# nico-bohlinger/RL-X

Measured on AMD Instinct MI355X. Metric: env-steps/sec (whole node) PPO 4096 envs at 1/2/4/8 MI355X, higher is better.
Workload: dtype f32

## Files before the change

### rl-x_amd/csrc/common.h

```cpp
#pragma once
#include <hip/hip_runtime.h>
#include <hip/hip_ext.h>
#include <stdint.h>
#include <cstring>
#include <cmath>
#include <string>
#include <vector>
#include <functional>
#include "../../include/rlx_hip.h"

namespace rlx {

void set_error(const std::string& msg);

#define RLX_HIP_TRY(expr)                                                                      \
  do {                                                                                         \
    hipError_t e_ = (expr);                                                                    \
    if (e_ != hipSuccess) {                                                                    \
      ::rlx::set_error(std::string(#expr) + " failed: " + hipGetErrorString(e_) + " (" __FILE__ \
                       ":" + std::to_string(__LINE__) + ")");                                  \
      return RLX_EHIP;                                                                         \
    }                                                                                          \
  } while (0)

// ... 37 lines not shown
  hipEvent_t e0, e1;
};
struct ProfRow {
  int kid, engine;
  int64_t M;
  int N, K;
  int64_t launches, timed;
  double ms, flops, bytes;
};
struct Twin { const void* p[4] = {nullptr, nullptr, nullptr, nullptr}; };

}

struct AttrOnce {
  uint64_t mask = 0;
  static int dev() { int d = 0; (void)hipGetDevice(&d); return d & 63; }
  bool done() const { return (mask >> dev()) & 1; }
  void mark() { mask |= 1ull << dev(); }
};

struct rlx_ctx {
  int device = 0;
  rlx::Scratch slots[3][rlx::SL_COUNT];
  int bank = 0;
  int opt_flip = 0;
  hipStream_t side = nullptr;
  hipEvent_t ev_fork = nullptr, ev_join = nullptr;
  hipEvent_t ev_rows[2] = {nullptr, nullptr};
  hipEvent_t ev_cdone[2] = {nullptr, nullptr};
  const float* dbg_sac_eps[2] = {nullptr, nullptr};
  bool l1fwd_mfma = true;
  bool pipeline_updates = true;
  bool pf_valid = false;
  uint32_t pf_key_in[2] = {0, 0}, pf_key_out[2] = {0, 0};
  int pf_E = 0, pf_scheme = 0;
  int64_t pf_B = 0;
  hipEvent_t pf_done = nullptr;
  hipEvent_t ev_perm_free = nullptr;
  bool perm_free_recorded = false;
  bool two_streams = true;
  const uint32_t* l1_xmax = nullptr;
  const uint32_t* xmax_slot[2] = {nullptr, nullptr};
  int lf_idle_cus = 0;
  bool dw_recompute = false;
  float* l12_stats = nullptr;
  bool l12_ran = false;
  bool dw_merge = true;
  void* dbg_stamps = nullptr;
  bool fwd2h = true;
  int gather_group_rows = 524288;
  bool gather_records = true;
  bool l12_fused = true;
  int ppo_tail = -1;
  int ppo_twin = -1;
  bool fused_recurrent_act = true;
  int num_cus = 256;
  void* defer = nullptr;
  bool prof_on = false;
  int prof_sample = 1;
  hipEvent_t prof_ref = nullptr;
  double prof_union_ms = 0.0;
  std::vector<rlx::ProfRec> prof_recs;
  std::vector<rlx::ProfRow> prof_rows;
  std::vector<hipEvent_t> prof_pool;
  bool gemm_bx = true;
  float bx_gscale = 1.f;
  bool adam_emit = true;
  bool bx_keep[3] = {false, false, false};
  struct RoImages { bool valid = false; const float* params[2] = {nullptr, nullptr}; const void* img[2][3] = {}; int nt[2][3] = {}; } ro_img;
  int bx_force_mi = 0;
  int bx_debug = 0;
  struct BxImage { const float* W; int trans, K, N; const void* img; };
  BxImage bx_img[3][32];
  int bx_n[3] = {0, 0, 0};
  bool disable_l1fused = false;
  std::vector<char> ro_nets_shadow;
  int rank = 0, world = 1;
  void* comm = nullptr;
  hipStream_t comm_stream = nullptr;
  hipEvent_t comm_ev[32] = {};
  int comm_ev_pos = 0;
  rlx_allreduce_fn ar_hook = nullptr;
  void* ar_hook_user = nullptr;
  int ro_exit = 0;
  int64_t bx_window_fallbacks = 0;
  int64_t ar_calls = 0;
  hipStream_t sac_st[2] = {nullptr, nullptr};
  hipEvent_t sac_ev[6] = {nullptr, nullptr, nullptr, nullptr, nullptr, nullptr};
  struct SacImages {
    bool valid = false; const float *pp = nullptr, *qp = nullptr, *qt = nullptr; rlx_mlp_desc pd{}, qd{}; int64_t np = 0, nq2 = 0;
    void written(const float* p, int64_t n) {
      if (!valid) return;
      auto hit = [&](const float* b, int64_t m) { return b && p < b + m && b < p + n; };
      if (hit(pp, np) || hit(qp, nq2) || hit(qt, nq2)) valid = false;
    }
  } sac_img;
  const void* sac_img_arena = nullptr;
  int sac_twin = 1;
  float* sched_host[4] = {nullptr, nullptr, nullptr, nullptr};
  hipEvent_t sched_ev[4] = {nullptr, nullptr, nullptr, nullptr};
  size_t sched_cap = 0;
  int sched_pos = 0;
  int espo_chunk = 2;
  int32_t* espo_host = nullptr;
  hipEvent_t espo_ev[3] = {nullptr, nullptr, nullptr};
  bool pf_dist = false;
// ... 329 lines not shown
```

### rl-x_amd/csrc/core.hip

```cpp
#include "common.h"
#include <algorithm>
#include <cstdio>
#include <cstdlib>
#include <utility>

namespace rlx {

static thread_local std::string g_last_error;

void set_error(const std::string& msg) { g_last_error = msg; }

void* scratch(rlx_ctx* ctx, ScratchSlot s, size_t bytes) {
  Scratch& sl = ctx->slots[ctx->bank][s];
  if (sl.bytes >= bytes && sl.ptr) return sl.ptr;
  if (sl.ptr) {
    if (hipDeviceSynchronize() != hipSuccess) { set_error("hipDeviceSynchronize failed in scratch()"); return nullptr; }
    (void)hipFree(sl.ptr);
    sl.ptr = nullptr;
    sl.bytes = 0;
  }
  size_t want = ((bytes > (size_t(1) << 20) ? bytes + bytes / 8 : bytes) + 255) & ~size_t(255);
  void* p = nullptr;
  hipError_t e = hipMalloc(&p, want);
  if (e != hipSuccess) {
// ... 153 lines not shown
      if (q.engine != rlx::PROF_ENGINE_HBM && ctx->prof_ref && hipEventElapsedTime(&t0, ctx->prof_ref, r.e0) == hipSuccess)
        iv.emplace_back(t0, t0 + ms);
    }
    ctx->prof_pool.push_back(r.e0);
    ctx->prof_pool.push_back(r.e1);
  }
  ctx->prof_recs.clear();
  std::sort(iv.begin(), iv.end());
  double uni = 0.0;
  float cs = 0.f, ce = -1.f;
  for (auto& p : iv) {
    if (ce < 0.f || p.first > ce) { if (ce >= 0.f) uni += ce - cs; cs = p.first; ce = p.second; }
    else if (p.second > ce) ce = p.second;
  }
  if (ce >= 0.f) uni += ce - cs;
  ctx->prof_union_ms = uni;
  return RLX_OK;
}

int rlx_prof_rows(rlx_ctx* ctx, rlx_prof_row* rows, int capacity, int* n_out) {
  RLX_REQUIRE(ctx && n_out && (rows || capacity == 0), RLX_EINVAL, "rlx_prof_rows: NULL pointer");
  const int n = (int)ctx->prof_rows.size();
  *n_out = n;
  for (int i = 0; i < n && i < capacity; ++i) {
    const rlx::ProfRow& q = ctx->prof_rows[i];
    rows[i] = rlx_prof_row{q.kid, q.engine, q.N, q.K, q.M, q.launches, q.timed, q.ms, q.flops, q.bytes};
  }
  return RLX_OK;
}

int rlx_prof_union_ms(rlx_ctx* ctx, double* out) {
  RLX_REQUIRE(ctx && out, RLX_EINVAL, "rlx_prof_union_ms: NULL pointer");
  *out = ctx->prof_union_ms;
  return RLX_OK;
}

int rlx_dbg_set_option(rlx_ctx* ctx, const char* name, int value) {
  RLX_REQUIRE(ctx && name, RLX_EINVAL, "rlx_dbg_set_option: NULL");
  if (std::string(name) == "sac_twin") { ctx->sac_twin = value; return RLX_OK; }
  if (std::string(name) == "disable_l1fused") { ctx->disable_l1fused = value != 0; return RLX_OK; }
  if (std::string(name) == "l1fwd_mfma") { ctx->l1fwd_mfma = value != 0; return RLX_OK; }
  if (std::string(name) == "pipeline_updates") { ctx->pipeline_updates = value != 0; return RLX_OK; }
  if (std::string(name) == "two_streams") { ctx->two_streams = value != 0; return RLX_OK; }
  if (std::string(name) == "ppo_twin") { ctx->ppo_twin = value; return RLX_OK; }
  if (std::string(name) == "ro_exit") { ctx->ro_exit = value; return RLX_OK; }
  if (std::string(name) == "lf_idle_cus") { ctx->lf_idle_cus = value < 0 ? 0 : value; return RLX_OK; }
  if (std::string(name) == "dw_recompute") { ctx->dw_recompute = value != 0; return RLX_OK; }
  if (std::string(name) == "dw_merge") { ctx->dw_merge = value != 0; return RLX_OK; }
  if (std::string(name) == "fwd2h") { ctx->fwd2h = value != 0; return RLX_OK; }
  if (std::string(name) == "l12_fused") { ctx->l12_fused = value != 0; return RLX_OK; }
  if (std::string(name) == "gather_group_rows") { ctx->gather_group_rows = value; return RLX_OK; }
  if (std::string(name) == "gather_records") { ctx->gather_records = value != 0; return RLX_OK; }
  if (std::string(name) == "ppo_tail") { ctx->ppo_tail = value < 0 ? -1 : (value > 2 ? 2 : value); return RLX_OK; }
  if (std::string(name) == "bx_force_mi") { ctx->bx_force_mi = value; return RLX_OK; }
  if (std::string(name) == "adam_emit") { ctx->adam_emit = value != 0; return RLX_OK; }
  if (std::string(name) == "bx_debug") { ctx->bx_debug = value; return RLX_OK; }
  if (std::string(name) == "bx_gscale_log2") { ctx->bx_gscale = ldexpf(1.f, value < 0 ? 0 : (value > 40 ? 40 : value)); return RLX_OK; }
  if (std::string(name) == "gemm_bx") { ctx->gemm_bx = value != 0; return RLX_OK; }
  if (std::string(name) == "prof_sample") { ctx->prof_sample = value < 1 ? 1 : value; return RLX_OK; }
  if (std::string(name) == "espo_chunk") { ctx->espo_chunk = value < 1 ? 1 : value; return RLX_OK; }
  if (std::string(name) == "fused_recurrent_act") { ctx->fused_recurrent_act = value != 0; return RLX_OK; }
  RLX_REQUIRE(false, RLX_EINVAL, "rlx_dbg_set_option: unknown option");
}

int rlx_dbg_get_counter(rlx_ctx* ctx, const char* name, int64_t* out) {
  RLX_REQUIRE(ctx && name && out, RLX_EINVAL, "rlx_dbg_get_counter: NULL");
  int bank = 0, slot = 0;
  if (sscanf(name, "scratch_ptr:%d:%d", &bank, &slot) == 2 && bank >= 0 && bank < 3 && slot >= 0 && slot < rlx::SL_COUNT) {
    *out = (int64_t)reinterpret_cast<uintptr_t>(ctx->slots[bank][slot].ptr);
    return RLX_OK;
  }
  if (sscanf(name, "scratch_bytes:%d:%d", &bank, &slot) == 2 && bank >= 0 && bank < 3 && slot >= 0 && slot < rlx::SL_COUNT) {
    *out = (int64_t)ctx->slots[bank][slot].bytes;
    return RLX_OK;
  }
  if (std::string(name) == "allreduce_calls") { *out = ctx->ar_calls; return RLX_OK; }
  if (std::string(name) == "bx_window_fallbacks") { *out = ctx->bx_window_fallbacks; return RLX_OK; }
  if (std::string(name) == "gemm_bx") { *out = ctx->gemm_bx ? 1 : 0; return RLX_OK; }
  RLX_REQUIRE(false, RLX_EINVAL, "rlx_dbg_get_counter: unknown counter");
}

int rlx_version(void) { return 200; }

const char* rlx_last_error(void) { return rlx::g_last_error.c_str(); }

int rlx_ctx_create(int device, rlx_ctx** out) {
  RLX_REQUIRE(out != nullptr, RLX_EINVAL, "rlx_ctx_create: out is NULL");
  int count = 0;
  RLX_HIP_TRY(hipGetDeviceCount(&count));
  RLX_REQUIRE(device >= 0 && device < count, RLX_EINVAL, "rlx_ctx_create: no such HIP device");
  RLX_HIP_TRY(hipSetDevice(device));
  hipDeviceProp_t prop;
  RLX_HIP_TRY(hipGetDeviceProperties(&prop, device));
  rlx_ctx* c = new rlx_ctx();
  c->device = device;
  c->num_cus = prop.multiProcessorCount;
  if (const char* e = getenv("RLX_GEMM_BX")) c->gemm_bx = atoi(e) != 0;
  if (const char* e = getenv("RLX_BX_DEBUG")) c->bx_debug = atoi(e);
  *out = c;
  return RLX_OK;
}

int rlx_dist_release(rlx_ctx* ctx);

int rlx_ctx_destroy(rlx_ctx* ctx) {
  if (!ctx) return RLX_OK;
// ... 40 lines not shown
```

### rl-x_amd/csrc/ppo.hip

```cpp
#include "ppo_internal.h"
#include "gemm_bx.h"
#include "dist.h"

namespace rlx {

constexpr float LOG_2PI = 1.8378770664093453f;
constexpr float HALF_LOG_2PIE = 1.4189385332046727f;
constexpr int HEAD_ROWS = 64;

__global__ __launch_bounds__(256) void k_gather(const float* __restrict__ states, const float* __restrict__ actions,
                                                const float* __restrict__ logp, const float* __restrict__ returns,
                                                const float* __restrict__ adv, const int32_t* __restrict__ idx,
                                                float* __restrict__ mb_x, float* __restrict__ mb_a,
                                                float* __restrict__ aux, const int32_t* __restrict__ valid_rows,
                                                int64_t mb, int O, int A, const float* __restrict__ cstates,
                                                float* __restrict__ mb_xc, int Oc) {
  const int64_t nv = valid_rows ? (int64_t)*valid_rows : mb;
  const int64_t nx = mb * O, na = mb * A, nxc = cstates ? mb * Oc : 0;
  const int64_t total = nx + na + mb + nxc;
  for (int64_t e = (int64_t)blockIdx.x * 256 + threadIdx.x; e < total; e += (int64_t)gridDim.x * 256) {
    if (e >= nx + na + mb) {
      const int64_t f = e - nx - na - mb;
      const int64_t r = f / Oc;
      const int d = (int)(f - r * Oc);
// ... 837 lines not shown
    }
  }
  __syncthreads();
  {
    constexpr int nk3 = K / X_BK;
    auto loadT = [&](int kt, float4 (&rr)[2]) {
      const int kk = (kt < nk3 ? kt : nk3 - 1) * X_BK;
#pragma unroll
      for (int p = 0; p < 2; ++p) rr[p] = *reinterpret_cast<const float4*>(T + (a_r + 32 * p) * TL_TS + kk + a_c);
    };
    const float so2 = X_WINV / gs;
    const int ntc = N2 / G_BN;
    for (int nt = 0; nt < ntc; ++nt) {
      f32x16 acc[1][2];
#pragma unroll
      for (int j = 0; j < 2; ++j)
#pragma unroll
        for (int rr = 0; rr < 16; ++rr) acc[0][j][rr] = 0.f;
      bx_kloop<1>(planes, n.W3t, nk3, ntc * 4, nt * 4 + wn * 2, wm, lane, a_r, a_c, loadT, acc, gs);
      const int64_t off = (m0 + wm * 32 + 4 * (lane >> 5)) * N2 + nt * G_BN + wn * 64 + (lane & 31);
      const float* hsb = n.H2 + off;
      float* cb = n.dZ2 + off;
      float hh[2][16];
#pragma unroll
      for (int j = 0; j < 2; ++j)
#pragma unroll
        for (int rr = 0; rr < 16; ++rr) hh[j][rr] = hsb[(int64_t)((rr & 3) + 8 * (rr >> 2)) * N2 + j * 32];
#pragma unroll
      for (int j = 0; j < 2; ++j)
#pragma unroll
        for (int rr = 0; rr < 16; ++rr)
          cb[(int64_t)((rr & 3) + 8 * (rr >> 2)) * N2 + j * 32] = acc[0][j][rr] * so2 * act_grad_t<ACT>(hh[j][rr]);
    }
  }
}

template <int ACT>
__global__ __launch_bounds__(256, 2) void k_tail_bx(TailNet p, TailNet c, const float* __restrict__ mb_a,
                                                    const float* __restrict__ aux, const double* __restrict__ stats,
                                                    float* __restrict__ metrics, int64_t M, int N2, float inv_mb, float clip,
                                                    float ent_coef, float critic_coef, const int32_t* __restrict__ valid_rows,
                                                    float gs, int both, int which) {
  extern __shared__ __attribute__((aligned(16))) char tl_smem[];
  const bool critic = both ? blockIdx.y != 0 : which != 0;
  if (!critic)
    tail_body<true, ACT>(p, tl_smem, mb_a, aux, stats, metrics, M, N2, inv_mb, clip, ent_coef, critic_coef, valid_rows, gs);
  else
    tail_body<false, ACT>(c, tl_smem, mb_a, aux, stats, metrics, M, N2, inv_mb, clip, ent_coef, critic_coef, valid_rows, gs);
}

#ifndef RLX_T32_PFC
#define RLX_T32_PFC 2
#endif
constexpr int T32_ROWS = 32;
template <bool POLICY, int ACT, int N2>
__device__ __forceinline__ void tail32_body(const TailNet& n, char* __restrict__ smem, const float* __restrict__ mb_a,
                                            const float* __restrict__ aux, const double* __restrict__ stats,
                                            float* __restrict__ metrics, int64_t M, float inv_mb, float clip, float ent_coef,
                                            float critic_coef, const int32_t* __restrict__ valid_rows, float gs) {
  constexpr int K = TL_K3, AP = 8, NP = 2, RP = T32_ROWS / NP, KQ = K / 8;
  constexpr int HROW = 2 * N2 + 16, HPL = T32_ROWS * HROW;
  constexpr int DROW = 2 * K + 16, DPL = T32_ROWS * DROW;
  constexpr int TREG = (T32_ROWS * TL_TS * 4 > 2 * DPL) ? T32_ROWS * TL_TS * 4 : 2 * DPL;
  char* H2P = smem;
  float* T = reinterpret_cast<float*>(smem + 2 * HPL);
  char* D3P = smem + 2 * HPL;
  float* Ws = reinterpret_cast<float*>(smem + 2 * HPL + TREG);
  float* Ds = Ws + K * AP;
  float* DLs = Ds + T32_ROWS * AP;
  float* red = DLs + T32_ROWS * AP;
  const int t = threadIdx.x, lane = t & 63, w = t >> 6, li = lane & 31, lh = lane >> 5;
  const int64_t m0 = (int64_t)blockIdx.x * T32_ROWS;
  const int A = n.A, PS = n.PS;
  {
    constexpr int NV = T32_ROWS * N2 / 4 / 256;
    float4 hv[NV];
    const int sr = t >> 3, sc = (t & 7) * 4;
    const float* hp = n.H2 + (m0 + sr) * N2 + sc;
#pragma unroll
    for (int i = 0; i < NV; ++i) hv[i] = *reinterpret_cast<const float4*>(hp + 32 * i);
    for (int i = t; i < K * AP; i += 256) {
      const int k = i >> 3, a = i & 7;
      Ws[i] = a < A ? n.Wh[k * A + a] : 0.f;
    }
    char* d0 = H2P + sr * HROW + sc * 2;
#pragma unroll
    for (int i = 0; i < NV; ++i) {
      uint32_t a0, a1, b0, b1;
      bx_split2(hv[i].x * X_ASCALE, hv[i].y * X_ASCALE, a0, a1);
      bx_split2(hv[i].z * X_ASCALE, hv[i].w * X_ASCALE, b0, b1);
      *reinterpret_cast<u32x2*>(d0 + 64 * i) = u32x2{a0, b0};
      *reinterpret_cast<u32x2*>(d0 + 64 * i + HPL) = u32x2{a1, b1};
    }
  }
  __syncthreads();
  {
    f32x16 acc;
#pragma unroll
    for (int r = 0; r < 16; ++r) acc[r] = 0.f;
    constexpr int NB = N2 / 16, PF = 4;
    const char* ard = H2P + li * HROW + lh * 16;
    const u32x4* wf = n.W3f + (int64_t)w * X_NP * 64 + lane;
    constexpr int wstep = 4 * X_NP * 64;
    u32x4 bq[PF][X_NP];
#pragma unroll
    for (int u = 0; u < PF; ++u)
#pragma unroll
      for (int p = 0; p < X_NP; ++p) bq[u][p] = wf[(int64_t)u * wstep + p * 64];
#define T32_BLOCK(QU, REFILL)                                                                                         \
  {                                                                                                                   \
    u32x4 av[X_NP];                                                                                                   \
    _Pragma("unroll") for (int p = 0; p < X_NP; ++p) av[p] = *reinterpret_cast<const u32x4*>(ard + (QU) * 32 + p * HPL); \
    acc = __builtin_amdgcn_mfma_f32_32x32x16_f16(__builtin_bit_cast(f16x8, av[0]), __builtin_bit_cast(f16x8, bq[u][1]), acc, 0, 0, 0); \
    acc = __builtin_amdgcn_mfma_f32_32x32x16_f16(__builtin_bit_cast(f16x8, av[1]), __builtin_bit_cast(f16x8, bq[u][0]), acc, 0, 0, 0); \
    acc = __builtin_amdgcn_mfma_f32_32x32x16_f16(__builtin_bit_cast(f16x8, av[0]), __builtin_bit_cast(f16x8, bq[u][0]), acc, 0, 0, 0); \
    if (REFILL) {                                                                                                     \
      _Pragma("unroll") for (int p = 0; p < X_NP; ++p) bq[u][p] = wf[(int64_t)((QU) + PF) * wstep + p * 64];           \
    }                                                                                                                 \
    __builtin_amdgcn_sched_barrier(0);                                                                                \
  }
#pragma unroll 1
    for (int q = 0; q < NB - PF; q += PF) {
#pragma unroll
      for (int u = 0; u < PF; ++u) T32_BLOCK(q + u, true)
    }
#pragma unroll
    for (int u = 0; u < PF; ++u) T32_BLOCK(NB - PF + u, false)
#undef T32_BLOCK
    const float so = X_AINV * X_WINV, bv = n.b3[w * 32 + li];
    float* tb = T + (4 * lh) * TL_TS + w * 32 + li;
#pragma unroll
    for (int r = 0; r < 16; ++r) tb[((r & 3) + 8 * (r >> 2)) * TL_TS] = act_fwd_t<ACT>(fmaf(acc[r], so, bv));
  }
  __syncthreads();
  const int r = t >> 3, q8 = t & 7;
  const int64_t row = m0 + r;
  const bool valid = row < (valid_rows ? (int64_t)*valid_rows : M);
  float bias[AP], ls[AP];
#pragma unroll
  for (int a = 0; a < AP; ++a) {
    bias[a] = a < A ? n.bh[a] : 0.f;
    ls[a] = (POLICY && a < A) ? n.logstd[a] : 0.f;
  }
  hl_f4 h[KQ / 4];
  {
    const hl_f4* hp = reinterpret_cast<const hl_f4*>(T + r * TL_TS + q8 * KQ);
#pragma unroll
    for (int j = 0; j < KQ / 4; ++j) h[j] = hp[j];
  }
  float out[AP];
#pragma unroll
  for (int a = 0; a < AP; ++a) out[a] = 0.f;
#pragma unroll
  for (int j = 0; j < KQ / 4; ++j)
#pragma unroll
    for (int e = 0; e < 4; ++e) {
      const float* wr = Ws + (q8 * KQ + 4 * j + e) * AP;
      const hl_f4 w0 = *reinterpret_cast<const hl_f4*>(wr), w1 = *reinterpret_cast<const hl_f4*>(wr + 4);
      const float hv = h[j][e];
#pragma unroll
      for (int a = 0; a < 4; ++a) { out[a] = fmaf(hv, w0[a], out[a]); out[4 + a] = fmaf(hv, w1[a], out[4 + a]); }
    }
#pragma unroll
  for (int a = 0; a < AP; ++a) {
    out[a] += dpp_f(out[a], 0);
    out[a] += dpp_f(out[a], 1);
    out[a] += dpp_f(out[a], 2);
    out[a] += bias[a];
  }
  float d[AP], m0s = 0.f, m1s = 0.f, m2s = 0.f;
#pragma unroll
  for (int a = 0; a < AP; ++a) d[a] = 0.f;
  if (POLICY) {
    float nlp = 0.f, zs[AP], isd[AP];
#pragma unroll
    for (int a = 0; a < AP; ++a) {
      isd[a] = 1.0f / expf(ls[a]);
      const float act_a = (valid && a < A) ? mb_a[row * A + a] : out[a];
      zs[a] = (act_a - out[a]) * isd[a];
      if (a < A) nlp += -0.5f * zs[a] * zs[a] - 0.5f * LOG_2PI - ls[a];
    }
    float amean, ainv, astd;
    adv_norm_from_stats(stats, amean, ainv, astd);
    const float logp_old = valid ? aux[row * 3 + 0] : 0.f;
    const float advn = valid ? (aux[row * 3 + 2] - amean) * ainv : 0.f;
    const float logratio = valid ? nlp - logp_old : 0.f;
    const float ratio = expf(logratio);
    const float pg1 = -advn * ratio;
    const float rc = fminf(fmaxf(ratio, 1.f - clip), 1.f + clip);
    const float pg2 = -advn * rc;
    const bool inside = (ratio >= 1.f - clip) && (ratio <= 1.f + clip);
    const float d_ratio = (inside || pg1 > pg2) ? -advn : 0.f;
    const float d_logp = valid ? d_ratio * ratio * inv_mb : 0.f;
#pragma unroll
    for (int a = 0; a < AP; ++a) {
      d[a] = a < A ? d_logp * zs[a] * isd[a] : 0.f;
      if (q8 == 0) DLs[r * AP + a] = a < A ? d_logp * (zs[a] * zs[a] - 1.f) - (valid ? ent_coef * inv_mb : 0.f) : 0.f;
    }
    if (valid && q8 == 0) {
      m0s = fmaxf(pg1, pg2);
      m1s = (ratio - 1.f) - logratio;
      m2s = fabsf(ratio - 1.f) > clip ? 1.f : 0.f;
    }
    if (blockIdx.x == 0 && t == 0) {
      float ent = 0.f, sstd = 0.f;
      for (int a = 0; a < A; ++a) { ent += ls[a] + HALF_LOG_2PIE; sstd += expf(ls[a]); }
      metrics[2] = ent;
      metrics[5] = amean;
      metrics[6] = astd;
      metrics[7] = sstd / (float)A;
    }
  } else {
    if (valid) {
      const float diff = out[0] - aux[row * 3 + 1];
      if (q8 == 0) m0s = 0.5f * diff * diff;
      d[0] = critic_coef * inv_mb * diff;
    }
  }
  if (q8 == 0) {
#pragma unroll
    for (int a = 0; a < AP; ++a) Ds[r * AP + a] = d[a];
  }
  m0s = wave_sum(m0s);
  m1s = wave_sum(m1s);
  m2s = wave_sum(m2s);
  if ((t & 63) == 0) { red[(t >> 6) * 4 + 0] = m0s; red[(t >> 6) * 4 + 1] = m1s; red[(t >> 6) * 4 + 2] = m2s; }
  __syncthreads();
  float* pw = n.partials + (int64_t)blockIdx.x * PS;
  if (t == 0) {
    float* pm = pw + K * A + 2 * A;
    pm[0] = (red[0] + red[4]) + (red[8] + red[12]);
    pm[1] = (red[1] + red[5]) + (red[9] + red[13]);
    pm[2] = (red[2] + red[6]) + (red[10] + red[14]);
  }
  __syncthreads();
  {
    const int k = t % K, part = t / K;
    float dw[AP];
#pragma unroll
    for (int a = 0; a < AP; ++a) dw[a] = 0.f;
    for (int rr = part * RP; rr < (part + 1) * RP; ++rr) {
      const float hv = T[rr * TL_TS + k];
      const hl_f4 d0 = *reinterpret_cast<const hl_f4*>(Ds + rr * AP), d1 = *reinterpret_cast<const hl_f4*>(Ds + rr * AP + 4);
#pragma unroll
      for (int a = 0; a < 4; ++a) { dw[a] = fmaf(hv, d0[a], dw[a]); dw[4 + a] = fmaf(hv, d1[a], dw[4 + a]); }
    }
#pragma unroll
    for (int a = 0; a < AP; ++a) red[(part * K + k) * AP + a] = dw[a];
    __syncthreads();
    if (part == 0) {
#pragma unroll
      for (int a = 0; a < AP; ++a) dw[a] += red[(K + k) * AP + a];
      for (int a = 0; a < A; ++a) pw[k * A + a] = dw[a];
    }
  }
  if (t < A) {
    float sb = 0.f, sl = 0.f;
    for (int rr = 0; rr < T32_ROWS; ++rr) {
      sb += Ds[rr * AP + t];
      if (POLICY) sl += DLs[rr * AP + t];
    }
    pw[K * A + t] = sb;
    pw[K * A + A + t] = sl;
  }
  __syncthreads();
  {
    hl_f4* gp = reinterpret_cast<hl_f4*>(n.dZ3 + row * K + q8 * KQ);
    char* dp = D3P + r * DROW + q8 * KQ * 2;
#pragma unroll
    for (int j = 0; j < KQ / 4; ++j) {
      hl_f4 o;
#pragma unroll
      for (int e = 0; e < 4; ++e) {
        const float* wr = Ws + (q8 * KQ + 4 * j + e) * AP;
        const hl_f4 w0 = *reinterpret_cast<const hl_f4*>(wr), w1 = *reinterpret_cast<const hl_f4*>(wr + 4);
        float sacc = 0.f;
#pragma unroll
        for (int a = 0; a < 4; ++a) { sacc = fmaf(d[a], w0[a], sacc); sacc = fmaf(d[4 + a], w1[a], sacc); }
        o[e] = sacc * act_grad_t<ACT>(h[j][e]);
      }
      gp[j] = o;
      uint32_t a0, a1, b0, b1;
      bx_split2(o[0] * gs, o[1] * gs, a0, a1);
      bx_split2(o[2] * gs, o[3] * gs, b0, b1);
      *reinterpret_cast<u32x2*>(dp + 8 * j) = u32x2{a0, b0};
      *reinterpret_cast<u32x2*>(dp + 8 * j + DPL) = u32x2{a1, b1};
    }
  }
  __syncthreads();
  {
    constexpr int NTC = N2 / 32, JW = NTC / 4;
    f32x16 acc[JW];
#pragma unroll
    for (int j = 0; j < JW; ++j)
#pragma unroll
      for (int rr = 0; rr < 16; ++rr) acc[j][rr] = 0.f;
    const char* ard = D3P + li * DROW + lh * 16;
    const u32x4* wt = n.W3t + (int64_t)(w * JW) * X_NP * 64 + lane;
    constexpr int wstep = NTC * X_NP * 64;
    constexpr int PFC = RLX_T32_PFC, NBC = K / 16;
    u32x4 bc[PFC][JW][X_NP];
#pragma unroll
    for (int u = 0; u < PFC; ++u)
#pragma unroll
      for (int j = 0; j < JW; ++j)
#pragma unroll
        for (int p = 0; p < X_NP; ++p) bc[u][j][p] = wt[(int64_t)u * wstep + (j * X_NP + p) * 64];
#define T32C_BLOCK(QU, REFILL)                                                                                        \
  {                                                                                                                   \
    u32x4 av[X_NP];                                                                                                   \
    _Pragma("unroll") for (int p = 0; p < X_NP; ++p) av[p] = *reinterpret_cast<const u32x4*>(ard + (QU) * 32 + p * DPL); \
    _Pragma("unroll") for (int j = 0; j < JW; ++j) {                                                                  \
      acc[j] = __builtin_amdgcn_mfma_f32_32x32x16_f16(__builtin_bit_cast(f16x8, av[0]), __builtin_bit_cast(f16x8, bc[u][j][1]), acc[j], 0, 0, 0); \
      acc[j] = __builtin_amdgcn_mfma_f32_32x32x16_f16(__builtin_bit_cast(f16x8, av[1]), __builtin_bit_cast(f16x8, bc[u][j][0]), acc[j], 0, 0, 0); \
      acc[j] = __builtin_amdgcn_mfma_f32_32x32x16_f16(__builtin_bit_cast(f16x8, av[0]), __builtin_bit_cast(f16x8, bc[u][j][0]), acc[j], 0, 0, 0); \
    }                                                                                                                 \
    if (REFILL) {                                                                                                     \
      _Pragma("unroll") for (int j = 0; j < JW; ++j) _Pragma("unroll") for (int p = 0; p < X_NP; ++p)                  \
          bc[u][j][p] = wt[(int64_t)((QU) + PFC) * wstep + (j * X_NP + p) * 64];                                       \
    }                                                                                                                 \
    __builtin_amdgcn_sched_barrier(0);                                                                                \
  }
    static_assert(NBC % PFC == 0 && NBC >= PFC, "phase C: whole groups of PFC blocks");
#pragma unroll 1
    for (int q = 0; q < NBC - PFC; q += PFC) {
#pragma unroll
      for (int u = 0; u < PFC; ++u) T32C_BLOCK(q + u, true)
    }
#pragma unroll
    for (int u = 0; u < PFC; ++u) T32C_BLOCK(NBC - PFC + u, false)
#undef T32C_BLOCK
    const float so2 = X_WINV / gs;
#pragma unroll
    for (int j = 0; j < JW; ++j) {
      const int col = (w * JW + j) * 32 + li;
      float* cb = n.dZ2 + (m0 + 4 * lh) * N2 + col;
      const char* hb = H2P + (4 * lh) * HROW + col * 2;
#pragma unroll
      for (int rr = 0; rr < 16; ++rr) {
        const int rho = (rr & 3) + 8 * (rr >> 2);
        const _Float16 hi = *reinterpret_cast<const _Float16*>(hb + rho * HROW);
        const _Float16 lo = *reinterpret_cast<const _Float16*>(hb + rho * HROW + HPL);
        const float h2 = ((float)hi + (float)lo) * X_AINV;
        cb[(int64_t)rho * N2] = acc[j][rr] * so2 * act_grad_t<ACT>(h2);
      }
    }
  }
}

template <int ACT, int N2>
__global__ __launch_bounds__(256, 2) void k_tail32_bx(TailNet p, TailNet c, const float* __restrict__ mb_a,
                                                      const float* __restrict__ aux, const double* __restrict__ stats,
                                                      float* __restrict__ metrics, int64_t M, float inv_mb, float clip,
                                                      float ent_coef, float critic_coef, const int32_t* __restrict__ valid_rows,
                                                      float gs, int both, int which) {
  extern __shared__ __attribute__((aligned(16))) char tl32_smem[];
  const bool critic = both ? blockIdx.y != 0 : which != 0;
  if (!critic)
    tail32_body<true, ACT, N2>(p, tl32_smem, mb_a, aux, stats, metrics, M, inv_mb, clip, ent_coef, critic_coef, valid_rows, gs);
  else
    tail32_body<false, ACT, N2>(c, tl32_smem, mb_a, aux, stats, metrics, M, inv_mb, clip, ent_coef, critic_coef, valid_rows, gs);
}

static inline int tail_rows(const rlx_ctx* ctx, int N2, int act, int64_t mb) {
  const bool can32 = N2 == 256 && act == RLX_ACT_ELU && mb % T32_ROWS == 0;
  const bool want32 = ctx->ppo_tail == 2 || (ctx->ppo_tail < 0 && (mb <= 8192 || mb > 16384));
  return (can32 && want32) ? T32_ROWS : HEAD_ROWS;
}

static bool tail_shape_ok(const rlx_ctx* ctx, const rlx_mlp_desc& d, int64_t mb, const rlx_ppo_hparams& hp) {
  return ctx->ppo_tail && ctx->gemm_bx && !hp.discrete_actions && d.n_hidden == 3 && d.hidden[2] == TL_K3 && d.hidden[1] % G_BN == 0 &&
         d.hidden[1] <= 512 && d.out_dim <= 8 && mb >= 4096 && mb % HEAD_ROWS == 0;
}

static int launch_tail(rlx_ctx* ctx, const TailNet* p, const TailNet* c, const MbScratch& s, float* metrics, int64_t mb, int N2,
                       int mb_global, const rlx_ppo_hparams& hp, int act, hipStream_t st) {
  const TailNet dummy{};
  const TailNet& tp = p ? *p : dummy;
  const TailNet& tc = c ? *c : dummy;
  const int both = (p && c) ? 1 : 0, which = p ? 0 : 1;
  const float gs = bx_grad_scale(mb_global);
  const float inv_mb = 1.0f / (float)mb_global;
  const size_t lds = 2 * X_OPER + (size_t)HEAD_ROWS * TL_TS * sizeof(float);
  const double nets = both ? 2.0 : 1.0;
  ProfScope prof(s.valid_rows ? nullptr : ctx, PK_TAIL, nets * 4.0 * (double)mb * N2 * TL_K3, st,
                 nets * 4.0 * ((double)mb * (2 * N2 + TL_K3) + 2.0 * N2 * TL_K3), mb, TL_K3, N2, 1);
  if (tail_rows(ctx, N2, act, mb) == T32_ROWS) {
    constexpr int HPL = T32_ROWS * (2 * 256 + 16), DPL = T32_ROWS * (2 * TL_K3 + 16);
    constexpr int TREG = (T32_ROWS * TL_TS * 4 > 2 * DPL) ? T32_ROWS * TL_TS * 4 : 2 * DPL;
    const size_t lds32 = 2 * HPL + TREG + ((size_t)TL_K3 * 8 + 2 * T32_ROWS * 8 + 16 + 2 * TL_K3 * 8) * sizeof(float);
    static AttrOnce attr32;
    if (!attr32.done()) {
      RLX_HIP_TRY(hipFuncSetAttribute(reinterpret_cast<const void*>(k_tail32_bx<RLX_ACT_ELU, 256>),
                                      hipFuncAttributeMaxDynamicSharedMemorySize, 160 * 1024));
      attr32.mark();
    }
    RLX_PLAUNCH((k_tail32_bx<RLX_ACT_ELU, 256>), dim3((unsigned)(mb / T32_ROWS), both ? 2 : 1), dim3(256), lds32, st, tp, tc, s.mb_a,
                s.aux, s.stats, metrics, mb, inv_mb, hp.clip_range, hp.entropy_coef, hp.critic_coef, s.valid_rows, gs, both, which);
    RLX_LAUNCH_CHECK();
    return RLX_OK;
  }
#define RLX_TAIL_LAUNCH(ACTV)                                                                                        \
  {                                                                                                                  \
    static AttrOnce attr_set;                                                                                          \
    if (!attr_set.done()) {                                                                                                 \
      RLX_HIP_TRY(hipFuncSetAttribute(reinterpret_cast<const void*>(k_tail_bx<ACTV>),                                \
                                      hipFuncAttributeMaxDynamicSharedMemorySize, 160 * 1024));                      \
      attr_set.mark();                                                                                                 \
    }                                                                                                                \
    RLX_PLAUNCH((k_tail_bx<ACTV>), dim3((unsigned)(mb / HEAD_ROWS), both ? 2 : 1), dim3(256), lds, st, tp, tc, s.mb_a, s.aux,   \
                s.stats, metrics, mb, N2, inv_mb, hp.clip_range, hp.entropy_coef, hp.critic_coef, s.valid_rows, gs, both,      \
                which);                                                                                              \
  }
  if (act == RLX_ACT_ELU) RLX_TAIL_LAUNCH(RLX_ACT_ELU)
  else if (act == RLX_ACT_TANH) RLX_TAIL_LAUNCH(RLX_ACT_TANH)
  else RLX_TAIL_LAUNCH(RLX_ACT_RELU)
#undef RLX_TAIL_LAUNCH
  RLX_LAUNCH_CHECK();
  return RLX_OK;
}

template <bool POLICY>
static int launch_head_loss(float* H, const float* W, const float* b, const float* logstd, const MbScratch& s, float* metrics,
                            int64_t mb, int K, int A, int PS, float inv_mb, const rlx_ppo_hparams& hp, int act, hipStream_t st,
                            rlx_ctx* prof_ctx = nullptr) {
  const int nb = div_up(mb, HEAD_ROWS);
  ProfScope prof(s.valid_rows ? nullptr : prof_ctx, PK_HEAD_LOSS, 0.0, st,
                 4.0 * ((double)mb * (2 * K + A + 3) + (double)nb * PS + (double)K * A), mb, K, A, PROF_ENGINE_HBM);
  if (POLICY && hp.discrete_actions) {
    RLX_REQUIRE(A >= 2 && A <= 8, RLX_EUNSUP, "ppo: the Categorical head supports 2..8 actions");
    const size_t ldsd = ((size_t)HEAD_ROWS * (K + 1) + (size_t)K * A + 2 * (size_t)HEAD_ROWS * A + 2 * A) * sizeof(float);
    RLX_REQUIRE(ldsd <= 160 * 1024, RLX_EUNSUP, "ppo head: last hidden layer too wide for the LDS-staged head kernel");
    hipLaunchKernelGGL((k_head_loss<POLICY, true>), dim3(nb), dim3(256), ldsd, st, H, W, b, logstd, s.mb_a, s.aux, s.stats,
                       s.head_part, metrics, mb, K, A, PS, inv_mb, hp.clip_range, hp.entropy_coef, hp.critic_coef, act,
                       s.valid_rows);
    RLX_LAUNCH_CHECK();
    return RLX_OK;
  }
  if (A <= 8 && (K == 64 || K == 128 || K == 256)) {
    const int NP = 256 / K > 0 ? 256 / K : 1;
    const size_t lds = ((size_t)K * 8 + 2 * HEAD_ROWS * 8 + (size_t)HEAD_ROWS * (K + 1) + (size_t)NP * K * 8 + 16) * sizeof(float);
#define RLX_HL_FAST(KQV)                                                                                        \
  {                                                                                                             \
    static AttrOnce attr_set;                                                                                     \
    if (!attr_set.done()) {                                                                                            \
      RLX_HIP_TRY(hipFuncSetAttribute(reinterpret_cast<const void*>(k_head_loss_fast<POLICY, KQV>),              \
                                      hipFuncAttributeMaxDynamicSharedMemorySize, 160 * 1024));                 \
      attr_set.mark();                                                                                            \
    }                                                                                                           \
    RLX_PLAUNCH((k_head_loss_fast<POLICY, KQV>), dim3(nb), dim3(256), lds, st, H, W, b, logstd, s.mb_a, s.aux,          \
                s.stats, s.head_part, metrics, mb, A, PS, inv_mb, hp.clip_range, hp.entropy_coef, hp.critic_coef,        \
// ... 1198 lines not shown
```

Measured before the change: 7.842 million.

## Run tail32 kernel with eight waves, using helper waves to prefetch weights and inputs

Adds an eight-wave variant of the 32-row PPO tail kernel and makes it the default. The main four waves still run the MFMA work, while the extra four preload the head weights, biases and the W3t prologue fragments, and the main waves load per-row actions, logp and advantage before the first barrier. The dZ3 backward-to-hidden step is spread over all 512 threads. The intent is to hide global-load latency and raise parallelism, at the cost of more registers per block, lower occupancy limits (launch bounds change) and idle helper waves during the compute phases. Optional clock-stamp instrumentation is added behind a compile flag.

Measured after the change: 7.954 million (median of 6 runs). 1.01x the previous value.

```diff
diff --git a/rl-x_amd/csrc/common.h b/rl-x_amd/csrc/common.h
--- a/rl-x_amd/csrc/common.h
+++ b/rl-x_amd/csrc/common.h
@@ -113,6 +113,7 @@
   bool gather_records = true;
   bool l12_fused = true;
   int ppo_tail = -1;
+  int tail32_waves = 8;
   int ppo_twin = -1;
   bool fused_recurrent_act = true;
   int num_cus = 256;
diff --git a/rl-x_amd/csrc/core.hip b/rl-x_amd/csrc/core.hip
--- a/rl-x_amd/csrc/core.hip
+++ b/rl-x_amd/csrc/core.hip
@@ -229,6 +229,11 @@
   if (std::string(name) == "gather_group_rows") { ctx->gather_group_rows = value; return RLX_OK; }
   if (std::string(name) == "gather_records") { ctx->gather_records = value != 0; return RLX_OK; }
   if (std::string(name) == "ppo_tail") { ctx->ppo_tail = value < 0 ? -1 : (value > 2 ? 2 : value); return RLX_OK; }
+  if (std::string(name) == "tail32_waves") {
+    RLX_REQUIRE(value == 4 || value == 8, RLX_EINVAL, "rlx_dbg_set_option: tail32_waves is 4 or 8");
+    ctx->tail32_waves = value;
+    return RLX_OK;
+  }
   if (std::string(name) == "bx_force_mi") { ctx->bx_force_mi = value; return RLX_OK; }
   if (std::string(name) == "adam_emit") { ctx->adam_emit = value != 0; return RLX_OK; }
   if (std::string(name) == "bx_debug") { ctx->bx_debug = value; return RLX_OK; }
diff --git a/rl-x_amd/csrc/ppo.hip b/rl-x_amd/csrc/ppo.hip
--- a/rl-x_amd/csrc/ppo.hip
+++ b/rl-x_amd/csrc/ppo.hip
@@ -913,13 +913,19 @@
 #ifndef RLX_T32_PFC
 #define RLX_T32_PFC 2
 #endif
+#ifndef RLX_T32_STAMPS
+#define RLX_T32_STAMPS 0
+#endif
 constexpr int T32_ROWS = 32;
-template <bool POLICY, int ACT, int N2>
+template <bool POLICY, int ACT, int N2, int NWV>
 __device__ __forceinline__ void tail32_body(const TailNet& n, char* __restrict__ smem, const float* __restrict__ mb_a,
                                             const float* __restrict__ aux, const double* __restrict__ stats,
                                             float* __restrict__ metrics, int64_t M, float inv_mb, float clip, float ent_coef,
-                                            float critic_coef, const int32_t* __restrict__ valid_rows, float gs) {
+                                            float critic_coef, const int32_t* __restrict__ valid_rows, float gs,
+                                            unsigned long long* __restrict__ stamps) {
+  static_assert(NWV == 4 || NWV == 8, "tail32: four or eight waves per tile");
   constexpr int K = TL_K3, AP = 8, NP = 2, RP = T32_ROWS / NP, KQ = K / 8;
+  constexpr int NT = 64 * NWV, TPR = NT / T32_ROWS;
   constexpr int HROW = 2 * N2 + 16, HPL = T32_ROWS * HROW;
   constexpr int DROW = 2 * K + 16, DPL = T32_ROWS * DROW;
   constexpr int TREG = (T32_ROWS * TL_TS * 4 > 2 * DPL) ? T32_ROWS * TL_TS * 4 : 2 * DPL;
@@ -930,19 +936,44 @@
   float* Ds = Ws + K * AP;
   float* DLs = Ds + T32_ROWS * AP;
   float* red = DLs + T32_ROWS * AP;
+  float* BL = red + NP * K * AP;
   const int t = threadIdx.x, lane = t & 63, w = t >> 6, li = lane & 31, lh = lane >> 5;
   const int64_t m0 = (int64_t)blockIdx.x * T32_ROWS;
   const int A = n.A, PS = n.PS;
+  const bool hw = NWV == 4 || __builtin_amdgcn_readfirstlane(w) < 4;
+#if RLX_T32_STAMPS
+#define T32_STAMP(I) if (stamps && t == 0 && blockIdx.x == 0 && blockIdx.y == 0) stamps[I] = clock64();
+#define T32_WALL(I) if (stamps && t == 0 && blockIdx.x == 0 && blockIdx.y == 0) stamps[I] = wall_clock64();
+#else
+#define T32_STAMP(I)
+#define T32_WALL(I)
+#endif
+  T32_STAMP(0)
+  T32_WALL(14)
+  constexpr int NTC = N2 / 32, JW = NTC / NWV;
+  constexpr int PFC = RLX_T32_PFC * (NWV / 4), NBC = K / 16, wstepC = NTC * X_NP * 64;
+  const u32x4* wt = n.W3t + (int64_t)(w * JW) * X_NP * 64 + lane;
+  u32x4 bc[PFC][JW][X_NP];
+  auto c_prologue = [&]() {
+#pragma unroll
+    for (int u = 0; u < PFC; ++u)
+#pragma unroll
+      for (int j = 0; j < JW; ++j)
+#pragma unroll
+        for (int p = 0; p < X_NP; ++p) bc[u][j][p] = wt[(int64_t)u * wstepC + (j * X_NP + p) * 64];
+  };
   {
-    constexpr int NV = T32_ROWS * N2 / 4 / 256;
+    constexpr int NV = T32_ROWS * N2 / 4 / NT;
     float4 hv[NV];
-    const int sr = t >> 3, sc = (t & 7) * 4;
+    const int sr = t / TPR, sc = (t % TPR) * 4;
     const float* hp = n.H2 + (m0 + sr) * N2 + sc;
 #pragma unroll
-    for (int i = 0; i < NV; ++i) hv[i] = *reinterpret_cast<const float4*>(hp + 32 * i);
-    for (int i = t; i < K * AP; i += 256) {
-      const int k = i >> 3, a = i & 7;
-      Ws[i] = a < A ? n.Wh[k * A + a] : 0.f;
+    for (int i = 0; i < NV; ++i) hv[i] = *reinterpret_cast<const float4*>(hp + 4 * TPR * i);
+    if (NWV == 4) {
+      for (int i = t; i < K * AP; i += 256) {
+        const int k = i >> 3, a = i & 7;
+        Ws[i] = a < A ? n.Wh[k * A + a] : 0.f;
+      }
     }
     char* d0 = H2P + sr * HROW + sc * 2;
 #pragma unroll
@@ -950,12 +981,47 @@
       uint32_t a0, a1, b0, b1;
       bx_split2(hv[i].x * X_ASCALE, hv[i].y * X_ASCALE, a0, a1);
       bx_split2(hv[i].z * X_ASCALE, hv[i].w * X_ASCALE, b0, b1);
-      *reinterpret_cast<u32x2*>(d0 + 64 * i) = u32x2{a0, b0};
-      *reinterpret_cast<u32x2*>(d0 + 64 * i + HPL) = u32x2{a1, b1};
-    }
-  }
+      *reinterpret_cast<u32x2*>(d0 + 8 * TPR * i) = u32x2{a0, b0};
+      *reinterpret_cast<u32x2*>(d0 + 8 * TPR * i + HPL) = u32x2{a1, b1};
+    }
+  }
+  T32_STAMP(1)
   __syncthreads();
-  {
+  T32_STAMP(2)
+  const int r = t >> 3, q8 = t & 7;
+  const int64_t row = m0 + r;
+  float bias[AP], ls[AP];
+  float pre_act[AP], pre_lp = 0.f, pre_ret = 0.f, pre_adv = 0.f, amean = 0.f, ainv = 0.f, astd = 0.f, pre_b3 = 0.f;
+  bool pre_valid = false;
+  if (NWV == 8) {
+    if (hw) {
+      pre_valid = row < (valid_rows ? (int64_t)*valid_rows : M);
+      pre_b3 = n.b3[w * 32 + li];
+      if (POLICY) {
+#pragma unroll
+        for (int a = 0; a < AP; ++a) pre_act[a] = mb_a[row * A + (a < A ? a : A - 1)];
+      }
+      if (POLICY) {
+        adv_norm_from_stats(stats, amean, ainv, astd);
+        pre_lp = aux[row * 3 + 0];
+        pre_adv = aux[row * 3 + 2];
+      } else {
+        pre_ret = aux[row * 3 + 1];
+      }
+    } else {
+      c_prologue();
+      const int i0 = t - 256, a = i0 & 7, ac = a < A ? a : A - 1;
+      float wv[K * AP / 256], bl = 0.f;
+#pragma unroll
+      for (int u = 0; u < K * AP / 256; ++u) wv[u] = n.Wh[((i0 >> 3) + 32 * u) * A + ac];
+      if (i0 < AP) bl = n.bh[ac];
+      else if (POLICY && i0 < 2 * AP) bl = n.logstd[ac];
+#pragma unroll
+      for (int u = 0; u < K * AP / 256; ++u) Ws[i0 + 256 * u] = a < A ? wv[u] : 0.f;
+      if (i0 < 2 * AP) BL[i0] = a < A ? bl : 0.f;
+    }
+  }
+  if (hw) {
     f32x16 acc;
 #pragma unroll
     for (int r = 0; r < 16; ++r) acc[r] = 0.f;
@@ -988,22 +1054,26 @@
 #pragma unroll
     for (int u = 0; u < PF; ++u) T32_BLOCK(NB - PF + u, false)
 #undef T32_BLOCK
-    const float so = X_AINV * X_WINV, bv = n.b3[w * 32 + li];
+    T32_STAMP(3)
+    const float so = X_AINV * X_WINV, bv = NWV == 8 ? pre_b3 : n.b3[w * 32 + li];
     float* tb = T + (4 * lh) * TL_TS + w * 32 + li;
 #pragma unroll
     for (int r = 0; r < 16; ++r) tb[((r & 3) + 8 * (r >> 2)) * TL_TS] = act_fwd_t<ACT>(fmaf(acc[r], so, bv));
   }
+  T32_STAMP(4)
   __syncthreads();
-  const int r = t >> 3, q8 = t & 7;
-  const int64_t row = m0 + r;
-  const bool valid = row < (valid_rows ? (int64_t)*valid_rows : M);
-  float bias[AP], ls[AP];
+  T32_STAMP(5)
+  const bool valid = NWV == 8 ? pre_valid : row < (valid_rows ? (int64_t)*valid_rows : M);
 #pragma unroll
   for (int a = 0; a < AP; ++a) {
-    bias[a] = a < A ? n.bh[a] : 0.f;
-    ls[a] = (POLICY && a < A) ? n.logstd[a] : 0.f;
+    bias[a] = NWV == 8 ? BL[a] : (a < A ? n.bh[a] : 0.f);
+    ls[a] = NWV == 8 ? BL[AP + a] : ((POLICY && a < A) ? n.logstd[a] : 0.f);
   }
   hl_f4 h[KQ / 4];
+  float d[AP], m0s = 0.f, m1s = 0.f, m2s = 0.f;
+#pragma unroll
+  for (int a = 0; a < AP; ++a) d[a] = 0.f;
+  if (hw) {
   {
     const hl_f4* hp = reinterpret_cast<const hl_f4*>(T + r * TL_TS + q8 * KQ);
 #pragma unroll
@@ -1029,22 +1099,18 @@
     out[a] += dpp_f(out[a], 2);
     out[a] += bias[a];
   }
-  float d[AP], m0s = 0.f, m1s = 0.f, m2s = 0.f;
-#pragma unroll
-  for (int a = 0; a < AP; ++a) d[a] = 0.f;
   if (POLICY) {
     float nlp = 0.f, zs[AP], isd[AP];
 #pragma unroll
     for (int a = 0; a < AP; ++a) {
       isd[a] = 1.0f / expf(ls[a]);
-      const float act_a = (valid && a < A) ? mb_a[row * A + a] : out[a];
+      const float act_a = (valid && a < A) ? (NWV == 8 ? pre_act[a] : mb_a[row * A + a]) : out[a];
       zs[a] = (act_a - out[a]) * isd[a];
       if (a < A) nlp += -0.5f * zs[a] * zs[a] - 0.5f * LOG_2PI - ls[a];
     }
-    float amean, ainv, astd;
-    adv_norm_from_stats(stats, amean, ainv, astd);
-    const float logp_old = valid ? aux[row * 3 + 0] : 0.f;
-    const float advn = valid ? (aux[row * 3 + 2] - amean) * ainv : 0.f;
+    if (NWV == 4) adv_norm_from_stats(stats, amean, ainv, astd);
+    const float logp_old = valid ? (NWV == 8 ? pre_lp : aux[row * 3 + 0]) : 0.f;
+    const float advn = valid ? ((NWV == 8 ? pre_adv : aux[row * 3 + 2]) - amean) * ainv : 0.f;
     const float logratio = valid ? nlp - logp_old : 0.f;
     const float ratio = expf(logratio);
     const float pg1 = -advn * ratio;
@@ -1073,7 +1139,7 @@
     }
   } else {
     if (valid) {
-      const float diff = out[0] - aux[row * 3 + 1];
+      const float diff = out[0] - (NWV == 8 ? pre_ret : aux[row * 3 + 1]);
       if (q8 == 0) m0s = 0.5f * diff * diff;
       d[0] = critic_coef * inv_mb * diff;
     }
@@ -1086,6 +1152,8 @@
   m1s = wave_sum(m1s);
   m2s = wave_sum(m2s);
   if ((t & 63) == 0) { red[(t >> 6) * 4 + 0] = m0s; red[(t >> 6) * 4 + 1] = m1s; red[(t >> 6) * 4 + 2] = m2s; }
+  }
+  T32_STAMP(6)
   __syncthreads();
   float* pw = n.partials + (int64_t)blockIdx.x * PS;
   if (t == 0) {
@@ -1095,11 +1163,13 @@
     pm[2] = (red[2] + red[6]) + (red[10] + red[14]);
   }
   __syncthreads();
+  T32_STAMP(7)
   {
     const int k = t % K, part = t / K;
     float dw[AP];
 #pragma unroll
     for (int a = 0; a < AP; ++a) dw[a] = 0.f;
+    if (hw) {
     for (int rr = part * RP; rr < (part + 1) * RP; ++rr) {
       const float hv = T[rr * TL_TS + k];
       const hl_f4 d0 = *reinterpret_cast<const hl_f4*>(Ds + rr * AP), d1 = *reinterpret_cast<const hl_f4*>(Ds + rr * AP + 4);
@@ -1108,6 +1178,7 @@
     }
 #pragma unroll
     for (int a = 0; a < AP; ++a) red[(part * K + k) * AP + a] = dw[a];
+    }
     __syncthreads();
     if (part == 0) {
 #pragma unroll
@@ -1124,21 +1195,39 @@
     pw[K * A + t] = sb;
     pw[K * A + A + t] = sl;
   }
+  constexpr int CQ = K / TPR;
+  const int zr = NWV == 8 ? (t & 31) : t / TPR, zc = (NWV == 8 ? (t >> 5) : (t % TPR)) * CQ;
+  hl_f4 h3[CQ / 4];
+  float dd[AP];
+  if (NWV == 8) {
+    const hl_f4* hp = reinterpret_cast<const hl_f4*>(T + zr * TL_TS + zc);
+#pragma unroll
+    for (int j = 0; j < CQ / 4; ++j) h3[j] = hp[j];
+    const hl_f4 d0 = *reinterpret_cast<const hl_f4*>(Ds + zr * AP), d1 = *reinterpret_cast<const hl_f4*>(Ds + zr * AP + 4);
+#pragma unroll
+    for (int a = 0; a < 4; ++a) { dd[a] = d0[a]; dd[4 + a] = d1[a]; }
+    if (hw) c_prologue();
+  }
+  T32_STAMP(8)
   __syncthreads();
+  T32_STAMP(9)
   {
-    hl_f4* gp = reinterpret_cast<hl_f4*>(n.dZ3 + row * K + q8 * KQ);
-    char* dp = D3P + r * DROW + q8 * KQ * 2;
-#pragma unroll
-    for (int j = 0; j < KQ / 4; ++j) {
+    hl_f4* gp = reinterpret_cast<hl_f4*>(n.dZ3 + (m0 + zr) * K + zc);
+    char* dp = D3P + zr * DROW + zc * 2;
+#pragma unroll
+    for (int j = 0; j < CQ / 4; ++j) {
       hl_f4 o;
 #pragma unroll
       for (int e = 0; e < 4; ++e) {
-        const float* wr = Ws + (q8 * KQ + 4 * j + e) * AP;
+        const float* wr = Ws + (zc + 4 * j + e) * AP;
         const hl_f4 w0 = *reinterpret_cast<const hl_f4*>(wr), w1 = *reinterpret_cast<const hl_f4*>(wr + 4);
         float sacc = 0.f;
 #pragma unroll
-        for (int a = 0; a < 4; ++a) { sacc = fmaf(d[a], w0[a], sacc); sacc = fmaf(d[4 + a], w1[a], sacc); }
-        o[e] = sacc * act_grad_t<ACT>(h[j][e]);
+        for (int a = 0; a < 4; ++a) {
+          sacc = fmaf(NWV == 8 ? dd[a] : d[a], w0[a], sacc);
+          sacc = fmaf(NWV == 8 ? dd[4 + a] : d[4 + a], w1[a], sacc);
+        }
+        o[e] = sacc * act_grad_t<ACT>(NWV == 8 ? h3[j][e] : h[j][e]);
       }
       gp[j] = o;
       uint32_t a0, a1, b0, b1;
@@ -1148,25 +1237,18 @@
       *reinterpret_cast<u32x2*>(dp + 8 * j + DPL) = u32x2{a1, b1};
     }
   }
+  T32_STAMP(10)
   __syncthreads();
+  T32_STAMP(11)
   {
-    constexpr int NTC = N2 / 32, JW = NTC / 4;
     f32x16 acc[JW];
 #pragma unroll
     for (int j = 0; j < JW; ++j)
 #pragma unroll
       for (int rr = 0; rr < 16; ++rr) acc[j][rr] = 0.f;
     const char* ard = D3P + li * DROW + lh * 16;
-    const u32x4* wt = n.W3t + (int64_t)(w * JW) * X_NP * 64 + lane;
-    constexpr int wstep = NTC * X_NP * 64;
-    constexpr int PFC = RLX_T32_PFC, NBC = K / 16;
-    u32x4 bc[PFC][JW][X_NP];
-#pragma unroll
-    for (int u = 0; u < PFC; ++u)
-#pragma unroll
-      for (int j = 0; j < JW; ++j)
-#pragma unroll
-        for (int p = 0; p < X_NP; ++p) bc[u][j][p] = wt[(int64_t)u * wstep + (j * X_NP + p) * 64];
+    constexpr int wstep = wstepC;
+    if (NWV == 4) c_prologue();
 #define T32C_BLOCK(QU, REFILL)                                                                                        \
   {                                                                                                                   \
     u32x4 av[X_NP];                                                                                                   \
@@ -1191,6 +1273,7 @@
 #pragma unroll
     for (int u = 0; u < PFC; ++u) T32C_BLOCK(NBC - PFC + u, false)
 #undef T32C_BLOCK
+    T32_STAMP(12)
     const float so2 = X_WINV / gs;
 #pragma unroll
     for (int j = 0; j < JW; ++j) {
@@ -1207,20 +1290,24 @@
       }
     }
   }
-}
-
-template <int ACT, int N2>
-__global__ __launch_bounds__(256, 2) void k_tail32_bx(TailNet p, TailNet c, const float* __restrict__ mb_a,
+  T32_STAMP(13)
+  T32_WALL(15)
+#undef T32_STAMP
+#undef T32_WALL
+}
+
+template <int ACT, int N2, int NWV>
+__global__ __launch_bounds__(64 * NWV, NWV / 2) void k_tail32_bx(TailNet p, TailNet c, const float* __restrict__ mb_a,
                                                       const float* __restrict__ aux, const double* __restrict__ stats,
                                                       float* __restrict__ metrics, int64_t M, float inv_mb, float clip,
                                                       float ent_coef, float critic_coef, const int32_t* __restrict__ valid_rows,
-                                                      float gs, int both, int which) {
+                                                      float gs, int both, int which, unsigned long long* __restrict__ stamps) {
   extern __shared__ __attribute__((aligned(16))) char tl32_smem[];
   const bool critic = both ? blockIdx.y != 0 : which != 0;
   if (!critic)
-    tail32_body<true, ACT, N2>(p, tl32_smem, mb_a, aux, stats, metrics, M, inv_mb, clip, ent_coef, critic_coef, valid_rows, gs);
+    tail32_body<true, ACT, N2, NWV>(p, tl32_smem, mb_a, aux, stats, metrics, M, inv_mb, clip, ent_coef, critic_coef, valid_rows, gs, stamps);
   else
-    tail32_body<false, ACT, N2>(c, tl32_smem, mb_a, aux, stats, metrics, M, inv_mb, clip, ent_coef, critic_coef, valid_rows, gs);
+    tail32_body<false, ACT, N2, NWV>(c, tl32_smem, mb_a, aux, stats, metrics, M, inv_mb, clip, ent_coef, critic_coef, valid_rows, gs, stamps);
 }
 
 static inline int tail_rows(const rlx_ctx* ctx, int N2, int act, int64_t mb) {
@@ -1250,14 +1337,22 @@
     constexpr int HPL = T32_ROWS * (2 * 256 + 16), DPL = T32_ROWS * (2 * TL_K3 + 16);
     constexpr int TREG = (T32_ROWS * TL_TS * 4 > 2 * DPL) ? T32_ROWS * TL_TS * 4 : 2 * DPL;
     const size_t lds32 = 2 * HPL + TREG + ((size_t)TL_K3 * 8 + 2 * T32_ROWS * 8 + 16 + 2 * TL_K3 * 8) * sizeof(float);
-    static AttrOnce attr32;
-    if (!attr32.done()) {
-      RLX_HIP_TRY(hipFuncSetAttribute(reinterpret_cast<const void*>(k_tail32_bx<RLX_ACT_ELU, 256>),
-                                      hipFuncAttributeMaxDynamicSharedMemorySize, 160 * 1024));
-      attr32.mark();
-    }
-    RLX_PLAUNCH((k_tail32_bx<RLX_ACT_ELU, 256>), dim3((unsigned)(mb / T32_ROWS), both ? 2 : 1), dim3(256), lds32, st, tp, tc, s.mb_a,
-                s.aux, s.stats, metrics, mb, inv_mb, hp.clip_range, hp.entropy_coef, hp.critic_coef, s.valid_rows, gs, both, which);
+    unsigned long long* stamps = RLX_T32_STAMPS ? (unsigned long long*)ctx->dbg_stamps : nullptr;
+#define RLX_TAIL32_LAUNCH(NWV)                                                                                       \
+  {                                                                                                                  \
+    static AttrOnce attr32;                                                                                          \
+    if (!attr32.done()) {                                                                                            \
+      RLX_HIP_TRY(hipFuncSetAttribute(reinterpret_cast<const void*>(k_tail32_bx<RLX_ACT_ELU, 256, NWV>),             \
+                                      hipFuncAttributeMaxDynamicSharedMemorySize, 160 * 1024));                      \
+      attr32.mark();                                                                                                 \
+    }                                                                                                                \
+    RLX_PLAUNCH((k_tail32_bx<RLX_ACT_ELU, 256, NWV>), dim3((unsigned)(mb / T32_ROWS), both ? 2 : 1), dim3(64 * NWV), lds32, st, tp, \
+                tc, s.mb_a, s.aux, s.stats, metrics, mb, inv_mb, hp.clip_range, hp.entropy_coef, hp.critic_coef, s.valid_rows, gs,   \
+                both, which, stamps);                                                                                \
+  }
+    if (ctx->tail32_waves == 8) RLX_TAIL32_LAUNCH(8)
+    else RLX_TAIL32_LAUNCH(4)
+#undef RLX_TAIL32_LAUNCH
     RLX_LAUNCH_CHECK();
     return RLX_OK;
   }
```
